# roym899/sdfest

Hardware: AMD Instinct MI355X
Metric: depth renders/sec fwd+bwd, 640×480 @ 64³ SDF; grad max-abs-err vs ref (higher is better)
Workload: dtype f32

## Files before the change

sdfest_amd/csrc/device.hpp:

```cpp
#pragma once

#include "common.hpp"

namespace sdfr {
namespace {

__device__ __forceinline__ V3 pixel_ray(int row, int col, float cx, float cy, float rfx, float rfy) {
  const float dx = ((float)col + 0.5f - cx) * rfx;
  const float dy = -((float)row + 0.5f - cy) * rfy;
  const float inv_len = __builtin_amdgcn_rsqf(fmaf(dx, dx, fmaf(dy, dy, 1.0f)));
  return mk(dx * inv_len, dy * inv_len, -inv_len);
}

__device__ __forceinline__ V3 rot_t(const ViewSetup& s, V3 v) {
  return mk(fmaf(s.rot[0], v.x, fmaf(s.rot[3], v.y, s.rot[6] * v.z)),
            fmaf(s.rot[1], v.x, fmaf(s.rot[4], v.y, s.rot[7] * v.z)),
            fmaf(s.rot[2], v.x, fmaf(s.rot[5], v.y, s.rot[8] * v.z)));
}
__device__ __forceinline__ V3 rot_f(const ViewSetup& s, V3 v) {
  return mk(fmaf(s.rot[0], v.x, fmaf(s.rot[1], v.y, s.rot[2] * v.z)),
            fmaf(s.rot[3], v.x, fmaf(s.rot[4], v.y, s.rot[5] * v.z)),
            fmaf(s.rot[6], v.x, fmaf(s.rot[7], v.y, s.rot[8] * v.z)));
}

__device__ __forceinline__ float vmin(float a, float b) {
  float r;
  asm("v_min_f32 %0, %1, %2" : "=v"(r) : "v"(a), "v"(b));
  return r;
}
__device__ __forceinline__ float vmax(float a, float b) {
  float r;
  asm("v_max_f32 %0, %1, %2" : "=v"(r) : "v"(a), "v"(b));
  return r;
}

struct __attribute__((packed, aligned(4))) ZPair {
  float lo, hi;
};

struct Cell {
  float v[8];
  float ox, oy, oz;
  float bx, by, bz;
  int lin;
};

template <int RT>
__device__ __forceinline__ void gather_cell(const float* __restrict__ src, int R, float gx, float gy,
                                            float gz, Cell& c) {
  const int Rr = RT > 0 ? RT : R;
  const float top = (float)(Rr - 2);
  const float bx = fminf(fmaxf(floorf(gx), 0.0f), top);
  const float by = fminf(fmaxf(floorf(gy), 0.0f), top);
  const float bz = fminf(fmaxf(floorf(gz), 0.0f), top);
  c.ox = gx - bx; c.oy = gy - by; c.oz = gz - bz;
  c.bx = bx; c.by = by; c.bz = bz;
  const int lin = (Rr <= 256) ? (int)fmaf(fmaf(bx, (float)Rr, by), (float)Rr, bz)
                              : ((int)bx * Rr + (int)by) * Rr + (int)bz;
  c.lin = lin;
  const float* base = src + lin;
  const ZPair p00 = *reinterpret_cast<const ZPair*>(base);
  const ZPair p01 = *reinterpret_cast<const ZPair*>(base + Rr);
  const ZPair p10 = *reinterpret_cast<const ZPair*>(base + Rr * Rr);
  const ZPair p11 = *reinterpret_cast<const ZPair*>(base + Rr * Rr + Rr);
  c.v[0] = p00.lo; c.v[1] = p00.hi; c.v[2] = p01.lo; c.v[3] = p01.hi;
  c.v[4] = p10.lo; c.v[5] = p10.hi; c.v[6] = p11.lo; c.v[7] = p11.hi;
}

constexpr bool kRecordsBlocked = true;
__host__ __device__ __forceinline__ int record_slab(int R) {
  return kRecordsBlocked ? 4 * ((R + 1) >> 1) * ((R + 1) >> 1) : R * R;
}
__device__ __forceinline__ int record_index(int x, int y, int z, int Hb) {
  if (!kRecordsBlocked) return (x * (2 * Hb) + y) * (2 * Hb) + z;
  return (((x * Hb + (y >> 1)) * Hb + (z >> 1)) << 2) | ((y & 1) << 1) | (z & 1);
}

typedef int i32x4 __attribute__((ext_vector_type(4)));

typedef float f32x2 __attribute__((ext_vector_type(2)));
typedef int i32x2 __attribute__((ext_vector_type(2)));
__host__ __device__ __forceinline__ constexpr bool is_pow2(int v) { return v > 0 && (v & (v - 1)) == 0; }

template <int RT, bool PACKED>
__device__ __forceinline__ float march_sample(__amdgpu_buffer_rsrc_t src, int R, f32x2 gxy, float gz) {
  const int Rr = RT > 0 ? RT : R;
  const float top = (float)(Rr - 2), fR = (float)Rr;
  const f32x2 bxy = {fminf(fmaxf(floorf(gxy.x), 0.0f), top), fminf(fmaxf(floorf(gxy.y), 0.0f), top)};
  const float bz = fminf(fmaxf(floorf(gz), 0.0f), top);
  const f32x2 oxy = gxy - bxy, axy = 1.0f - oxy;
  const float oz = gz - bz, az = 1.0f - oz;
  const int lin = (Rr <= 256) ? (int)fmaf(fmaf(bxy.x, fR, bxy.y), fR, bz)
                              : ((int)bxy.x * Rr + (int)bxy.y) * Rr + (int)bz;
  f32x2 a01, a23, b01, b23;
  if (PACKED) {
    int rix;
    if (!kRecordsBlocked) {
      rix = lin;
    } else if (RT > 0 && is_pow2(RT) && RT >= 4) {
      constexpr int L = __builtin_ctz(RT > 0 ? RT : 2);
      constexpr int zhi = ((1 << L) - 2) << 1;
      int t;
      asm("v_bfi_b32 %0, %1, %2, %3" : "=v"(t) : "s"(zhi), "v"(lin << 1), "v"(lin));
      asm("v_bfi_b32 %0, 2, %1, %2" : "=v"(rix) : "v"(lin >> (L - 1)), "v"(t));
    } else {
      rix = record_index((int)bxy.x, (int)bxy.y, (int)bz, (Rr + 1) >> 1);
    }
    const i32x4 a = __builtin_amdgcn_raw_buffer_load_b128(src, rix * 16, 0, 0);
    const i32x4 b = __builtin_amdgcn_raw_buffer_load_b128(src, rix * 16, record_slab(Rr) * 16, 0);
    a01 = f32x2{__int_as_float(a.x), __int_as_float(a.y)};
    a23 = f32x2{__int_as_float(a.z), __int_as_float(a.w)};
    b01 = f32x2{__int_as_float(b.x), __int_as_float(b.y)};
    b23 = f32x2{__int_as_float(b.z), __int_as_float(b.w)};
  } else {
    const int off = lin * 4;
    const i32x2 p00 = __builtin_amdgcn_raw_buffer_load_b64(src, off, 0, 0);
    const i32x2 p01 = __builtin_amdgcn_raw_buffer_load_b64(src, off, Rr * 4, 0);
    const i32x2 p10 = __builtin_amdgcn_raw_buffer_load_b64(src, off, Rr * Rr * 4, 0);
    const i32x2 p11 = __builtin_amdgcn_raw_buffer_load_b64(src, off, (Rr * Rr + Rr) * 4, 0);
    a01 = f32x2{__int_as_float(p00.x), __int_as_float(p00.y)};
    a23 = f32x2{__int_as_float(p01.x), __int_as_float(p01.y)};
    b01 = f32x2{__int_as_float(p10.x), __int_as_float(p10.y)};
    b23 = f32x2{__int_as_float(p11.x), __int_as_float(p11.y)};
  }
  const f32x2 ox2 = {oxy.x, oxy.x}, ax2 = {axy.x, axy.x}, oy2 = {oxy.y, oxy.y}, ay2 = {axy.y, axy.y};
  const f32x2 c0 = __builtin_elementwise_fma(b01, ox2, a01 * ax2);
  const f32x2 c1 = __builtin_elementwise_fma(b23, ox2, a23 * ax2);
  const f32x2 c = __builtin_elementwise_fma(c1, oy2, c0 * ay2);
  return fmaf(c.y, oz, c.x * az);
}

__device__ __forceinline__ float trilerp(const Cell& c) {
  const float ax = 1.0f - c.ox, ay = 1.0f - c.oy, az = 1.0f - c.oz;
  const float c00 = fmaf(c.v[4], c.ox, c.v[0] * ax);
  const float c01 = fmaf(c.v[5], c.ox, c.v[1] * ax);
  const float c10 = fmaf(c.v[6], c.ox, c.v[2] * ax);
  const float c11 = fmaf(c.v[7], c.ox, c.v[3] * ax);
  const float c0 = fmaf(c10, c.oy, c00 * ay);
  const float c1 = fmaf(c11, c.oy, c01 * ay);
  return fmaf(c1, c.oz, c0 * az);
}

constexpr int kPatchWFwd = 8, kPatchWBwd = 16;
template <int PW> struct Patch {
  static constexpr int W = PW, H = 64 / PW, waves_x = kSubW / PW;
  static __device__ __forceinline__ int ox(int wave) { return (wave % waves_x) * W; }
  static __device__ __forceinline__ int oy(int wave) { return (wave / waves_x) * H; }
  static __device__ __forceinline__ int x(int lane) { return lane % W; }
  static __device__ __forceinline__ int y(int lane) { return lane / W; }
};
__device__ __forceinline__ float wave_sum(float v) {
#pragma unroll
  for (int off = 32; off >= 1; off >>= 1) v += __shfl_xor(v, off, 64);
  return v;
}

__device__ __forceinline__ float wave_sum8(const float (&v)[8], int lane) {
  const bool b5 = lane & 32, b4 = lane & 16, b3 = lane & 8;
  float a[4], b[2], c;
#pragma unroll
  for (int j = 0; j < 4; ++j) {
    const float keep = b5 ? v[j + 4] : v[j], send = b5 ? v[j] : v[j + 4];
    a[j] = keep + __shfl_xor(send, 32, 64);
  }
#pragma unroll
  for (int j = 0; j < 2; ++j) {
    const float keep = b4 ? a[j + 2] : a[j], send = b4 ? a[j] : a[j + 2];
    b[j] = keep + __shfl_xor(send, 16, 64);
  }
  {
    const float keep = b3 ? b[1] : b[0], send = b3 ? b[0] : b[1];
    c = keep + __shfl_xor(send, 8, 64);
  }
  c += __shfl_xor(c, 4, 64);
  c += __shfl_xor(c, 2, 64);
  c += __shfl_xor(c, 1, 64);
  return c;
}

constexpr int kFixedBits = 44;

__device__ __forceinline__ long long fixed_from_float(float x) {
  const double d = (double)x + 6755399441055744.0;
  return __double_as_longlong(d) - 0x4338000000000000LL;
}

template <int SHIFT, int SLOTS>
struct RunHash {
  static constexpr int kShift = SHIFT, kSlots = SLOTS, kLen = 1 << SHIFT;
  static constexpr int kBits = kFixedBits;
  static constexpr float kWeightLimit = 3.5e13f;
  unsigned long long vals[SLOTS << SHIFT];
  int keys[SLOTS];

  __device__ __forceinline__ void clear(int tid, int nthreads) {
    for (int i = tid; i < SLOTS; i += nthreads) keys[i] = -1;
    for (int i = tid; i < (SLOTS << SHIFT); i += nthreads) vals[i] = 0ull;
  }

  __device__ __forceinline__ int slot_of(int key) {
    unsigned h = (((unsigned)key * 2654435761u) >> 16) & (SLOTS - 1);
#pragma unroll 1
    for (int probe = 0; probe < 32; ++probe) {
      int cur = __builtin_nontemporal_load(&keys[h]);
      if (cur == -1) cur = atomicCAS(&keys[h], -1, key);
      if (cur == -1 || cur == key) return (int)h;
      h = (h + 1) & (SLOTS - 1);
    }
    return -1;
  }

  template <bool DET = false>
  __device__ __forceinline__ void add_one(float* __restrict__ gvol, int slot, int lin, float w,
                                          float to_fixed) {
    if (slot >= 0)
      atomicAdd(&vals[(slot << SHIFT) + (lin & (kLen - 1))], (unsigned long long)fixed_from_float(w * to_fixed));
    else if (DET)
      atomicAdd(reinterpret_cast<unsigned long long*>(gvol) + lin, (unsigned long long)fixed_from_float(w * to_fixed));
    else
      atomicAdd(gvol + lin, w);
  }

  template <bool DET = false>
  __device__ __forceinline__ void add_cell(float* __restrict__ gvol, int lin, int Rr,
                                           const float (&w)[8], float to_fixed) {
    const int col[4] = {lin, lin + Rr, lin + Rr * Rr, lin + Rr * Rr + Rr};
    int key[4], cur[4];
    unsigned h[4];
#pragma unroll
    for (int j = 0; j < 4; ++j) {
      key[j] = col[j] >> SHIFT;
      h[j] = (((unsigned)key[j] * 2654435761u) >> 16) & (SLOTS - 1);
      cur[j] = __builtin_nontemporal_load(&keys[h[j]]);
    }
    int slot[4];
#pragma unroll
    for (int j = 0; j < 4; ++j) slot[j] = (cur[j] == key[j]) ? (int)h[j] : slot_of(key[j]);
#pragma unroll
    for (int j = 0; j < 4; ++j) {
      add_one<DET>(gvol, slot[j], col[j], w[2 * j], to_fixed);
      const bool split = (col[j] & (kLen - 1)) == kLen - 1;
      const int s_hi = split ? slot_of(key[j] + 1) : slot[j];
      add_one<DET>(gvol, s_hi, col[j] + 1, w[2 * j + 1], to_fixed);
    }
  }

  template <bool DET = false>
  __device__ __forceinline__ void flush(float* __restrict__ gvol, int nvox, float from_fixed, int tid,
                                        int nthreads) {
    for (int i = tid; i < (SLOTS << SHIFT); i += nthreads) {
      const int key = keys[i >> SHIFT];
      if (key < 0) continue;
      const long long q = (long long)vals[i];
      const int lin = (key << SHIFT) + (i & (kLen - 1));
      if (q != 0 && lin < nvox) {
        if (DET) atomicAdd(reinterpret_cast<unsigned long long*>(gvol) + lin, (unsigned long long)q);
        else atomicAdd(gvol + lin, (float)q * from_fixed);
      }
    }
  }
};
template <int SLOTS>
struct PairRunHash {
  static constexpr int kSlots = SLOTS, kLen = 4;
  static constexpr int kBits = 22;
  static constexpr float kWeightLimit = 4194304.0f;
  unsigned long long vals[SLOTS * 4];
  int keys[SLOTS];

  __device__ __forceinline__ void clear(int tid, int nthreads) {
    typedef int i32x4v __attribute__((ext_vector_type(4)));
    i32x4v* k4 = reinterpret_cast<i32x4v*>(keys);
    i32x4v* v4 = reinterpret_cast<i32x4v*>(vals);
    for (int i = tid; i < SLOTS / 4; i += nthreads) k4[i] = i32x4v{-1, -1, -1, -1};
    for (int i = tid; i < SLOTS * 2; i += nthreads) v4[i] = i32x4v{0, 0, 0, 0};
  }

  __device__ __forceinline__ int slot_after(int key, unsigned h, int cur) {
#pragma unroll 1
    for (int probe = 0; probe < 32; ++probe) {
      if (cur == -1) cur = atomicCAS(&keys[h], -1, key);
      if (cur == -1 || cur == key) return (int)h;
      h = (h + 1) & (SLOTS - 1);
      cur = __builtin_nontemporal_load(&keys[h]);
    }
    return -1;
  }

  template <bool DET = false>
  __device__ __forceinline__ void add_cell(float* __restrict__ gvol, int lin, int Rr, const float (&w)[8],
                                           float to_fixed) {
    static_assert(!DET, "32-bit pair sums cannot hold the deterministic mode's quantum: use RunHash");
    const int col[4] = {lin, lin + Rr, lin + Rr * Rr, lin + Rr * Rr + Rr};
    int key[4], cur[4];
    unsigned h[4];
#pragma unroll
    for (int j = 0; j < 4; ++j) {
      key[j] = col[j] >> 2;
      h[j] = (((unsigned)key[j] * 2654435761u) >> 16) & (SLOTS - 1);
      cur[j] = __builtin_nontemporal_load(&keys[h[j]]);
    }
    int slot[4];
#pragma unroll
    for (int j = 0; j < 4; ++j) slot[j] = (cur[j] == key[j]) ? (int)h[j] : slot_after(key[j], h[j], cur[j]);
#pragma unroll
    for (int j = 0; j < 4; ++j) {
      if (slot[j] >= 0) {
        const long long lo = fixed_from_float(w[2 * j] * to_fixed), hi = fixed_from_float(w[2 * j + 1] * to_fixed);
        atomicAdd(&vals[slot[j] * 4 + (col[j] & 3)], (unsigned long long)(lo + (hi << 32)));
      } else {
        atomicAdd(gvol + col[j], w[2 * j]);
        atomicAdd(gvol + col[j] + 1, w[2 * j + 1]);
      }
    }
  }

  template <bool DET = false>
  __device__ __forceinline__ void flush(float* __restrict__ gvol, int nvox, float from_fixed, int tid, int nthreads) {
    static_assert(!DET, "use RunHash");
    for (int i = tid; i < SLOTS * 5; i += nthreads) {
      const int slot = i / 5, k = i - slot * 5;
      const int key = keys[slot];
      if (key < 0) continue;
      long long sum = 0;
      if (k < 4) sum += (long long)(int)(unsigned)(vals[slot * 4 + k] & 0xffffffffull);
      if (k > 0) {
        const long long q = (long long)vals[slot * 4 + k - 1];
        sum += (q - (long long)(int)(unsigned)((unsigned long long)q & 0xffffffffull)) >> 32;
      }
      const int lin = key * 4 + k;
      if (sum != 0 && lin < nvox) atomicAdd(gvol + lin, (float)sum * from_fixed);
    }
  }
};
using BatchHash = RunHash<2, 512>;
using SmallHash = RunHash<1, 1024>;

template <int CTRL> __device__ __forceinline__ int dpp_self(int v) {
  return __builtin_amdgcn_update_dpp(v, v, CTRL, 0xf, 0xf, false);
}
__device__ __forceinline__ int wave_min_to63(int v) {
  v = min(v, dpp_self<0x111>(v));
  v = min(v, dpp_self<0x112>(v));
  v = min(v, dpp_self<0x114>(v));
  v = min(v, dpp_self<0x118>(v));
  v = min(v, dpp_self<0x142>(v));
  v = min(v, dpp_self<0x143>(v));
  return v;
}
__device__ __forceinline__ int wave_max_to63(int v) {
  v = max(v, dpp_self<0x111>(v));
  v = max(v, dpp_self<0x112>(v));
  v = max(v, dpp_self<0x114>(v));
  v = max(v, dpp_self<0x118>(v));
  v = max(v, dpp_self<0x142>(v));
  v = max(v, dpp_self<0x143>(v));
  return v;
}

__device__ __forceinline__ float wave_max(float v) {
#pragma unroll
  for (int off = 32; off >= 1; off >>= 1) v = fmaxf(v, __shfl_xor(v, off, 64));
  return v;
}


}
}
```

sdfest_amd/csrc/render.hip:

```cpp
#include <algorithm>
#include <atomic>
#include <type_traits>

#include "common.hpp"
#include "device.hpp"
#include "sampler_device.hpp"


namespace sdfr {
namespace {

constexpr int kBlock = 256;
constexpr int kFwdWaves = SDFR_FWD_WAVES;
constexpr int kInlineSetupMaxViews = SDFR_INLINE_MAX_VIEWS;


__device__ __forceinline__ void setup_pose(int b, const float* __restrict__ pos, const float* __restrict__ quat,
                                           const float* __restrict__ inv_scale, int R, float fx, float fy,
                                           ViewSetup& s) {
  const float x = quat[4 * b], y = quat[4 * b + 1], z = quat[4 * b + 2], w = quat[4 * b + 3];
  const V3 p = mk(pos[3 * b], pos[3 * b + 1], pos[3 * b + 2]);
  const float isc = inv_scale[b];
  const float scale = 1.0f / isc;
  s.rot[0] = 1 - 2 * (y * y + z * z); s.rot[1] = 2 * (x * y - w * z);     s.rot[2] = 2 * (x * z + w * y);
// ... 50 lines not shown
            const unsigned long long m = __ballot(f);
            if (m) {
              if (first == R) first = i0 + __builtin_ctzll(m);
              last = i0 + 63 - __builtin_clzll(m);
            }
          }
        } else {
          for (int i = 0; i + 1 < R; ++i) {
            if (fminf(pm[i], pm[i + 1]) < vhit) {
              if (first == R) first = i;
              last = i;
            }
          }
        }
        if (last < 0) { empty = true; break; }
        lo[a] = fmaxf(-scale, ((float)first - 0.0625f) * cell - scale);
        hi[a] = fminf(scale, ((float)(last + 1) + 0.0625f) * cell - scale);
      }
    }
  }
  float umin = 3.0e38f, umax = -3.0e38f, vmin = 3.0e38f, vmax = -3.0e38f;
  bool in_front = true;
  auto corner = [&](int c) {
    const float sx = (c & 1) ? hi[0] : lo[0], sy = (c & 2) ? hi[1] : lo[1],
                sz = (c & 4) ? hi[2] : lo[2];
    const float X = p.x + s.rot[0] * sx + s.rot[1] * sy + s.rot[2] * sz;
    const float Y = p.y + s.rot[3] * sx + s.rot[4] * sy + s.rot[5] * sz;
    const float Z = p.z + s.rot[6] * sx + s.rot[7] * sy + s.rot[8] * sz;
    if (!(Z < -1e-6f)) in_front = false;
    const float iz = 1.0f / fmaxf(-Z, 1e-30f);
    const float u = cx + fx * X * iz;
    const float v = cy - fy * Y * iz;
    umin = fminf(umin, u); umax = fmaxf(umax, u);
    vmin = fminf(vmin, v); vmax = fmaxf(vmax, v);
  };
  if (WAVE) {
    corner(lane & 7);
#pragma unroll
    for (int off = 1; off <= 4; off <<= 1) {
      umin = fminf(umin, __shfl_xor(umin, off, 64)); umax = fmaxf(umax, __shfl_xor(umax, off, 64));
      vmin = fminf(vmin, __shfl_xor(vmin, off, 64)); vmax = fmaxf(vmax, __shfl_xor(vmax, off, 64));
    }
    in_front = __ballot(!in_front) == 0ull;
  } else {
    for (int c = 0; c < 8; ++c) corner(c);
  }
  int x0 = 0, y0 = 0, x1 = W, y1 = H;
  if (in_front) {
    const float mx = 2.0f + 1e-5f * fabsf(fx), my = 2.0f + 1e-5f * fabsf(fy);
    const float fx0 = fminf(fmaxf(floorf(umin - 0.5f - mx), 0.0f), (float)W);
    const float fx1 = fminf(fmaxf(ceilf(umax - 0.5f + mx) + 1.0f, 0.0f), (float)W);
    const float fy0 = fminf(fmaxf(floorf(vmin - 0.5f - my), 0.0f), (float)H);
    const float fy1 = fminf(fmaxf(ceilf(vmax - 0.5f + my) + 1.0f, 0.0f), (float)H);
    x0 = (int)fx0; x1 = (int)fx1; y0 = (int)fy0; y1 = (int)fy1;
  }
  if (empty) { x0 = y0 = x1 = y1 = 0; }
  s.rect[0] = x0; s.rect[1] = y0; s.rect[2] = x1; s.rect[3] = y1;
  if (WAVE && spans) {
    float cu[8], cv[8];
    float big = 0.0f;
#pragma unroll
    for (int c = 0; c < 8; ++c) {
      const float sx = (c & 1) ? hi[0] : lo[0], sy = (c & 2) ? hi[1] : lo[1], sz = (c & 4) ? hi[2] : lo[2];
      const float X = p.x + s.rot[0] * sx + s.rot[1] * sy + s.rot[2] * sz;
      const float Y = p.y + s.rot[3] * sx + s.rot[4] * sy + s.rot[5] * sz;
      const float Z = p.z + s.rot[6] * sx + s.rot[7] * sy + s.rot[8] * sz;
      const float iz = 1.0f / fmaxf(-Z, 1e-30f);
      cu[c] = cx + fx * X * iz;
      cv[c] = cy - fy * Y * iz;
      big = fmaxf(big, fmaxf(fabsf(cu[c]), fabsf(cv[c])));
    }
    bool sane = in_front && !empty && big < 4.0e4f && W <= 65535;
#pragma unroll
    for (int c = 0; c < 8; ++c) sane = sane && (cu[c] == cu[c]) && (cv[c] == cv[c]);
    s.spans = sane ? 1 : 0;
    const int rstride = resident_stride_words(H);
    if (sane || rr.row) {
      const float mx = 2.0f + 1e-5f * fabsf(fx), my = 2.0f + 1e-5f * fabsf(fy);
      const int nb = span_bands(H);
      float slope[12];
#pragma unroll
      for (int a = 0, e = 0; a < 8; ++a)
#pragma unroll
        for (int ax = 0; ax < 3; ++ax)
          if (!(a & (1 << ax))) {
            const int c2 = a | (1 << ax);
            slope[e++] = (cu[c2] - cu[a]) * __builtin_amdgcn_rcpf(cv[c2] - cv[a]);
          }
      for (int k0 = 0; k0 < nb; k0 += 64) {
        const int k = k0 + lane;
        const float ya = (float)(8 * k) + 0.5f - my, yb = (float)(8 * k) + 7.5f + my;
        float xmin = 3.0e38f, xmax = -3.0e38f;
        float da[8], db[8];
#pragma unroll
        for (int a = 0; a < 8; ++a) {
          da[a] = ya - cv[a];
          db[a] = yb - cv[a];
          const float u = (da[a] <= 0.0f && db[a] >= 0.0f) ? cu[a] : __int_as_float(0x7fc00000);
          xmin = fminf(xmin, u); xmax = fmaxf(xmax, u);
        }
#pragma unroll
        for (int a = 0, e = 0; a < 8; ++a)
#pragma unroll
          for (int ax = 0; ax < 3; ++ax)
            if (!(a & (1 << ax))) {
              const int c2 = a | (1 << ax);
              const float xa = (da[a] * da[c2] <= 0.0f) ? fmaf(da[a], slope[e], cu[a]) : __int_as_float(0x7fc00000);
              const float xb = (db[a] * db[c2] <= 0.0f) ? fmaf(db[a], slope[e], cu[a]) : __int_as_float(0x7fc00000);
              xmin = fminf(xmin, fminf(xa, xb)); xmax = fmaxf(xmax, fmaxf(xa, xb));
              ++e;
            }
        int sx0 = 0, sx1 = 0;
        if (!sane) {
          if (x1 > x0 && 8 * k < y1 && 8 * k + 8 > y0) { sx0 = x0; sx1 = x1; }
        } else if (xmin <= xmax && 8 * k < y1 && 8 * k + 8 > y0) {
          sx0 = max(x0, (int)fminf(fmaxf(floorf(xmin - 0.5f - mx), 0.0f), (float)W));
          sx1 = min(x1, (int)fminf(fmaxf(ceilf(xmax - 0.5f + mx) + 1.0f, 0.0f), (float)W));
          if (sx1 <= sx0) sx0 = sx1 = 0;
        }
        const unsigned word = (unsigned)sx0 | ((unsigned)sx1 << 16);
        if (k < nb) {
          if (sane) spans[k] = word;
          if (rr.row) {
            const unsigned prev = !rr.prev_ok ? kResidentClearAll : (k0 == 0 ? rr.prev0 : rr.row[2 * k]);
            rr.row[2 * k] = word;
            rr.row[2 * k + 1] = prev;
          }
        }
      }
      if (rr.row && lane == 0) {
        rr.row[rstride - 2] = rr.seq + 1u;
        rr.row[rstride - 1] = ~((rr.seq + 1u) ^ rr.key);
      }
    }
  }
  for (int k = 0; k < 3; ++k) {
    s.ep[k] = s.e[k] + scale;
    s.em[k] = s.e[k] - scale;
    s.tp[k] = s.e[k] + hi[k];
    s.tm[k] = s.e[k] + lo[k];
  }
}

template <bool WAVE = false>
__device__ __forceinline__ void compute_view_setup(int b, const float* __restrict__ pos,
                                                   const float* __restrict__ quat,
                                                   const float* __restrict__ inv_scale, int R, int W, int H,
                                                   float cx, float cy, float fx, float fy,
                                                   ViewSetup* __restrict__ out,
                                                   const float* __restrict__ plane_min = nullptr,
                                                   float threshold = 0.0f, unsigned* __restrict__ spans = nullptr,
                                                   ResidentRow rr = ResidentRow{}) {
  ViewSetup s;
  setup_pose(b, pos, quat, inv_scale, R, fx, fy, s);
  setup_box<WAVE>(s, R, W, H, cx, cy, fx, fy, plane_min, threshold,
                  spans ? spans + (size_t)b * span_stride_words(H) : nullptr, rr);
  if (!WAVE || (threadIdx.x & 63) == 0) out[b] = s;
}

__device__ __forceinline__ void count_close_view(unsigned* __restrict__ sync, int B, bool close,
                                                 unsigned long long* __restrict__ word) {
  const unsigned old = atomicAdd(&sync[2], 0x10000u | (close ? 1u : 0u));
  if ((old >> 16) + 1u != (unsigned)B) return;
  const unsigned c = (old & 0xffffu) + (close ? 1u : 0u);
  atomicExch(&sync[2], 0u);
  const unsigned seq = sync[4] + 1u;
  sync[4] = seq;
  sync[5] = c;
  if (word) __hip_atomic_store(word, ((unsigned long long)seq << 32) | c, __ATOMIC_RELAXED, __HIP_MEMORY_SCOPE_SYSTEM);
}

__device__ __forceinline__ ResidentRow resident_row(unsigned* __restrict__ rstate, int vouched, int b, int B, int W,
                                                    int H) {
  ResidentRow rr;
  if (rstate) {
    const int stride = resident_stride_words(H), lane = threadIdx.x & 63;
    rr.row = rstate + kResidentHeaderWords + (size_t)b * stride;
    rr.seq = rstate[0];
    rr.key = resident_key(B, W, H);
    const unsigned tag = rr.row[stride - 2], check = rr.row[stride - 1];
    rr.prev0 = lane < span_bands(H) ? rr.row[2 * lane] : 0u;
    rr.prev_ok = vouched != 0 && tag == rr.seq && check == ~(rr.seq ^ rr.key);
  }
  return rr;
}

__global__ void view_setup_kernel(const float* __restrict__ pos, const float* __restrict__ quat,
                                  const float* __restrict__ inv_scale, int B, int R, int W, int H,
                                  float cx, float cy, float fx, float fy,
                                  ViewSetup* __restrict__ out, const float* __restrict__ plane_min,
                                  float threshold, unsigned* __restrict__ spans, unsigned* __restrict__ rstate,
                                  int depth_resident) {
  const int b = blockIdx.x;
  if (b < B)
    compute_view_setup<true>(b, pos, quat, inv_scale, R, W, H, cx, cy, fx, fy, out, plane_min, threshold, spans,
                             resident_row(rstate, depth_resident, b, B, W, H));
}

struct PlaneEntry {
  unsigned long long a, b;
};
__device__ __forceinline__ void publish_plane_min(float* __restrict__ plane_min, PlaneEntry* __restrict__ ent,
                                                  unsigned tag, int j, float m) {
  if (ent) {
    const unsigned bits = __float_as_uint(m);
    __hip_atomic_store(&ent[j].a, ((unsigned long long)tag << 32) | bits, __ATOMIC_RELAXED, __HIP_MEMORY_SCOPE_AGENT);
    __hip_atomic_store(&ent[j].b, ((unsigned long long)tag << 32) | (unsigned)~bits, __ATOMIC_RELAXED,
                       __HIP_MEMORY_SCOPE_AGENT);
  } else {
    plane_min[j] = m;
  }
}

__device__ __forceinline__ void plane_min_block(const float* __restrict__ sdf, int R, int j,
                                                float* __restrict__ plane_min, PlaneEntry* __restrict__ ent = nullptr,
                                                unsigned tag = 0u) {
  __shared__ float red[4][4];
  const int axis = j / R, i = j % R, RR = R * R;
  const int tid = threadIdx.x;
  if (axis == 2 && (R & 3) == 0 && ((uintptr_t)sdf & 15) == 0) {
    if (i & 3) return;
    float m0 = 3.0e38f, m1 = 3.0e38f, m2 = 3.0e38f, m3 = 3.0e38f;
    for (int k = tid; k < RR; k += 256) {
      const float4 v = *reinterpret_cast<const float4*>(sdf + (size_t)k * R + i);
      m0 = fminf(m0, v.x); m1 = fminf(m1, v.y); m2 = fminf(m2, v.z); m3 = fminf(m3, v.w);
    }
#pragma unroll
    for (int off = 32; off >= 1; off >>= 1) {
      m0 = fminf(m0, __shfl_xor(m0, off, 64)); m1 = fminf(m1, __shfl_xor(m1, off, 64));
      m2 = fminf(m2, __shfl_xor(m2, off, 64)); m3 = fminf(m3, __shfl_xor(m3, off, 64));
    }
    if ((tid & 63) == 0) { red[tid >> 6][0] = m0; red[tid >> 6][1] = m1; red[tid >> 6][2] = m2; red[tid >> 6][3] = m3; }
    __syncthreads();
    if (tid < 4)
      publish_plane_min(plane_min, ent, tag, j + tid,
                        fminf(fminf(red[0][tid], red[1][tid]), fminf(red[2][tid], red[3][tid])));
    return;
  }
  float m = 3.0e38f;
  for (int k = tid; k < RR; k += 256) {
    const int u = k / R, v = k % R;
    const int idx = axis == 0 ? i * RR + k : (axis == 1 ? u * RR + i * R + v : k * R + i);
    m = fminf(m, sdf[idx]);
  }
#pragma unroll
  for (int off = 32; off >= 1; off >>= 1) m = fminf(m, __shfl_xor(m, off, 64));
  if ((tid & 63) == 0) red[tid >> 6][0] = m;
  __syncthreads();
  if (tid == 0) publish_plane_min(plane_min, ent, tag, j, fminf(fminf(red[0][0], red[1][0]), fminf(red[2][0], red[3][0])));
}

__global__ __launch_bounds__(256) void backward_prologue_kernel(
    float* __restrict__ g_sdf, size_t n_words, const float* __restrict__ pos,
    const float* __restrict__ quat, const float* __restrict__ inv_scale, int B, int R, int W, int H,
    float cx, float cy, float fx, float fy, ViewSetup* __restrict__ out) {
  const size_t i = (size_t)blockIdx.x * 256 + threadIdx.x;
  if (i < n_words) g_sdf[i] = 0.0f;
  if (i < (size_t)B) compute_view_setup((int)i, pos, quat, inv_scale, R, W, H, cx, cy, fx, fy, out);
}

__device__ __forceinline__ float4 min4(float4 a, float4 b) {
  return make_float4(fminf(a.x, b.x), fminf(a.y, b.y), fminf(a.z, b.z), fminf(a.w, b.w));
}
__device__ __forceinline__ void plane_min_fast_block(const float* __restrict__ sdf, int R, int blk,
                                                     PlaneEntry* __restrict__ ent, unsigned tag) {
  __shared__ float4 red4[4];
  const int tid = threadIdx.x, RR = R * R, Rq = R >> 2;
  const float4* v = reinterpret_cast<const float4*>(sdf);
  float4 m = make_float4(3.0e38f, 3.0e38f, 3.0e38f, 3.0e38f);
  const int axis = blk / R, i = blk - axis * R;
  if (axis == 0) {
    const float4* base = v + (size_t)i * (RR >> 2);
#pragma unroll 4
    for (int q = tid; q < (RR >> 2); q += 256) m = min4(m, base[q]);
  } else if (axis == 1) {
    const float4* base = v + (size_t)i * Rq;
#pragma unroll 4
    for (int q = tid; q < R * Rq; q += 256) m = min4(m, base[(size_t)(q / Rq) * (RR >> 2) + (q % Rq)]);
  } else {
    const int zq = i % Rq, part = i / Rq, rows = RR >> 2;
    const float4* base = v + (size_t)part * rows * Rq + zq;
#pragma unroll 4
    for (int r = tid; r < rows; r += 256) m = min4(m, base[(size_t)r * Rq]);
  }
#pragma unroll
  for (int off = 32; off >= 1; off >>= 1) {
    m.x = fminf(m.x, __shfl_xor(m.x, off, 64)); m.y = fminf(m.y, __shfl_xor(m.y, off, 64));
    m.z = fminf(m.z, __shfl_xor(m.z, off, 64)); m.w = fminf(m.w, __shfl_xor(m.w, off, 64));
  }
  if ((tid & 63) == 0) red4[tid >> 6] = m;
  __syncthreads();
  if (tid < 4) {
    const float4 a = min4(min4(red4[0], red4[1]), min4(red4[2], red4[3]));
    if (axis < 2) {
      if (tid == 0) publish_plane_min(nullptr, ent, tag, blk, fminf(fminf(a.x, a.y), fminf(a.z, a.w)));
    } else {
      const int zq = i % Rq, part = i / Rq;
      const float val = tid == 0 ? a.x : (tid == 1 ? a.y : (tid == 2 ? a.z : a.w));
      publish_plane_min(nullptr, ent, tag, 2 * R + part * R + 4 * zq + tid, val);
    }
  }
}

__device__ __forceinline__ void pack_cell(const float* __restrict__ sdf, int R, float4* __restrict__ cells, int lin) {
  const int RR = R * R;
  if (lin >= RR * R) return;
  const int z = lin % R, y = (lin / R) % R;
  if (y >= R - 1 || z >= R - 1) return;
  const float* p = sdf + lin;
  cells[record_index(lin / RR, y, z, (R + 1) >> 1)] = make_float4(p[0], p[1], p[R], p[R + 1]);
}

__global__ __launch_bounds__(256) void pack_cells_kernel(const float* __restrict__ sdf, int R,
                                                         float4* __restrict__ cells, int n_pack_blocks,
                                                         float* __restrict__ plane_min) {
  const int n_plane = (int)gridDim.x - n_pack_blocks;
  if ((int)blockIdx.x < n_plane) {
    plane_min_block(sdf, R, (int)blockIdx.x, plane_min);
    return;
  }
  pack_cell(sdf, R, cells, ((int)blockIdx.x - n_plane) * (int)blockDim.x + (int)threadIdx.x);
}

constexpr int kPrologueMaxPolls = 1 << 16;
__global__ __launch_bounds__(256) void forward_prologue_kernel(
    const float* __restrict__ sdf, int R, float4* __restrict__ cells, int n_plane, int n_setup,
    unsigned* __restrict__ sync, const float* __restrict__ pos, const float* __restrict__ quat,
    const float* __restrict__ inv_scale, int B, int W, int H, float cx, float cy, float fx, float fy,
    ViewSetup* __restrict__ out, float threshold, float* __restrict__ g_zero, size_t n_zero, int default_polls,
    unsigned* __restrict__ spans, unsigned* __restrict__ rstate, int depth_resident) {
  const unsigned tag = sync[0] + 1u;
  PlaneEntry* ent = reinterpret_cast<PlaneEntry*>(sync + kSyncHeaderWords);
  int blk = (int)blockIdx.x;
  if (blk < n_plane) {
    plane_min_fast_block(sdf, R, blk, ent, tag);
    return;
  }
  blk -= n_plane;
  if (blk < n_setup) {
    __shared__ float pm_s[6 * kPackedMaxR];
    const int tid = (int)threadIdx.x, n_ent = 6 * R;
    const int b = blk * 4 + (tid >> 6);
    ViewSetup s;
    ResidentRow rr;
    if (b < B) {
      setup_pose(b, pos, quat, inv_scale, R, fx, fy, s);
      rr = resident_row(rstate, depth_resident, b, B, W, H);
    }
    bool ready = false;
    const int max_polls = sync[6] == SDFR_SYNC_POLLS_MAGIC ? (int)sync[7] : default_polls;
    for (int poll = 0; poll < max_polls; ++poll) {
      bool ok = true;
      for (int j = tid; j < n_ent; j += 256) {
        const unsigned long long a = __hip_atomic_load(&ent[j].a, __ATOMIC_RELAXED, __HIP_MEMORY_SCOPE_AGENT);
        const unsigned long long c = __hip_atomic_load(&ent[j].b, __ATOMIC_RELAXED, __HIP_MEMORY_SCOPE_AGENT);
        const bool good = (unsigned)(a >> 32) == tag && (unsigned)(c >> 32) == tag && (unsigned)a == ~(unsigned)c;
        if (good) pm_s[j] = __uint_as_float((unsigned)a);
        ok = ok && good;
      }
      if (__syncthreads_and(ok)) { ready = true; break; }
      __builtin_amdgcn_s_sleep(1);
    }
    if (ready) {
      for (int z = tid; z < R; z += 256)
        pm_s[2 * R + z] = fminf(fminf(pm_s[2 * R + z], pm_s[3 * R + z]), fminf(pm_s[4 * R + z], pm_s[5 * R + z]));
      __syncthreads();
    }
    if (b < B) {
      setup_box<true>(s, R, W, H, cx, cy, fx, fy, ready ? pm_s : nullptr, threshold,
                      spans + (size_t)b * span_stride_words(H), rr);
      if ((tid & 63) == 0) {
        out[b] = s;
        if (!ready) atomicAdd(&sync[1], 1u);
      }
    }
    return;
  }
  blk -= n_setup;
  const int lin = blk * 256 + (int)threadIdx.x;
  const size_t vox = (size_t)R * R * R;
  for (size_t i = (size_t)lin; i < n_zero; i += vox) g_zero[i] = 0.0f;
  pack_cell(sdf, R, cells, lin);
}

struct Rect {
  int x0, y0, x1, y1;
};
__device__ __forceinline__ bool overlaps(const Rect& r, int px, int py, int w, int h) {
  return (px < r.x1) && (px + w > r.x0) && (py < r.y1) && (py + h > r.y0);
}

struct Ray {
  float dg[3];
  float t, tf;
  float inv_len;
  bool go;
};
template <bool TIGHT>
__device__ __forceinline__ Ray ray_setup(const ViewSetup& s, int row, int col, bool inside, float cx, float cy,
                                         float rfx, float rfy) {
  Ray r;
  const float dx = ((float)col + 0.5f - cx) * rfx;
  const float dy = -((float)row + 0.5f - cy) * rfy;
  const float inv_len = __builtin_amdgcn_rsqf(fmaf(dx, dx, fmaf(dy, dy, 1.0f)));
  const float ux = fmaf(s.rot[0], dx, fmaf(s.rot[3], dy, -s.rot[6]));
  const float uy = fmaf(s.rot[1], dx, fmaf(s.rot[4], dy, -s.rot[7]));
  const float uz = fmaf(s.rot[2], dx, fmaf(s.rot[5], dy, -s.rot[8]));
  const float dv[3] = {ux * inv_len, uy * inv_len, uz * inv_len};
  float t_near = -1e-10f, tf = 1e10f, t_near2 = -1e-10f, tf2 = 1e10f;
#pragma unroll
  for (int a = 0; a < 3; ++a) {
    const float inv = __builtin_amdgcn_rcpf(dv[a]);
    const float ta = s.ep[a] * inv, tb = s.em[a] * inv;
    t_near = vmax(t_near, vmin(ta, tb));
    if (TIGHT) {
      const float tc = s.tp[a] * inv, td = s.tm[a] * inv;
      t_near2 = vmax(t_near2, vmin(tc, td));
      tf2 = vmin(tf2, vmax(tc, td));
    } else {
      tf = vmin(tf, vmax(ta, tb));
    }
  }
  if (TIGHT) tf = tf2;
  const bool miss = !inside || (TIGHT ? ((t_near2 > tf2) || (tf2 < 0.0f)) : ((t_near > tf) || (tf < 0.0f)));
  r.t = vmax(t_near, 0.0f);
  r.tf = tf;
  r.inv_len = inv_len;
  r.go = !miss && (r.t < tf);
  const float kgrid = s.dgk;
  r.dg[0] = dv[0] * kgrid; r.dg[1] = dv[1] * kgrid; r.dg[2] = dv[2] * kgrid;
  return r;
}

template <int RT, bool PACKED, int SX, int SY, bool LOSS, bool TIGHT, int NW, bool RES = false>
__device__ __forceinline__ void forward_tile(
    int tile_x, int tile_y, int ntx, int nty, int b, const float* __restrict__ src, int R,
    long long src_view_stride, const ViewSetup& s, int W, int H, float cx, float cy,
    float rfx, float rfy, float threshold, int vec_ok, float* __restrict__ depth,
    const float* __restrict__ target, float* __restrict__ loss_part, const unsigned* __restrict__ spans,
    const unsigned* __restrict__ rrows = nullptr) {
  constexpr int kSubs = SX * SY, kTileW = SX * kSubW, kTileH = SY * kSubH;
  static_assert(kTileH == 8, "a forward tile is one band of the span array");
  constexpr int kThreads = NW * 64;
  using PF = Patch<kPatchWFwd>;
  const int px0 = tile_x * kTileW, py0 = tile_y * kTileH;
  float* img = depth + (size_t)b * H * W;
  const int tid = threadIdx.x;
  auto zero_fill = [&]() {
    typedef float f32x4 __attribute__((ext_vector_type(4)));
    const f32x4 zero4 = {0.0f, 0.0f, 0.0f, 0.0f};
    if (vec_ok) {
#pragma unroll
      for (int i = tid; i < kTileW * kTileH / 4; i += kThreads) {
        const int row = py0 + i / (kTileW / 4), col = px0 + (i % (kTileW / 4)) * 4;
        if (row < H && col < W) __builtin_nontemporal_store(zero4, reinterpret_cast<f32x4*>(img + (size_t)row * W + col));
      }
    } else {
      for (int i = tid; i < kTileW * kTileH; i += kThreads) {
        const int row = py0 + i / kTileW, col = px0 + i % kTileW;
        if (row < H && col < W) img[(size_t)row * W + col] = 0.0f;
      }
    }
  };
  uint2 band = make_uint2(0u, kResidentClearAll);
  if (RES && rrows) {
    band = *reinterpret_cast<const uint2*>(rrows + (size_t)b * resident_stride_words(H) + 2 * tile_y);
    if (!LOSS && !(px0 < (int)(band.x >> 16) && px0 + kTileW > (int)(band.x & 0xffffu))) {
      if (px0 < (int)(band.y >> 16) && px0 + kTileW > (int)(band.y & 0xffffu)) zero_fill();
      return;
    }
  }
  Rect rc{s.rect[0], s.rect[1], s.rect[2], s.rect[3]};
  const bool in_rect = overlaps(rc, px0, py0, kTileW, kTileH);
  if (RES && rrows) {
    rc.x0 = (int)(band.x & 0xffffu);
    rc.x1 = (int)(band.x >> 16);
  } else if (s.spans) {
    const unsigned sp = spans[(size_t)b * span_stride_words(H) + tile_y];
    rc.x0 = (int)(sp & 0xffffu);
    rc.x1 = (int)(sp >> 16);
  }

  if (!overlaps(rc, px0, py0, kTileW, kTileH)) {
    if (LOSS && in_rect && tid < kLossRec) loss_part[(((size_t)b * nty + tile_y) * ntx + tile_x) * kLossRec + tid] = 0.0f;
    if (px0 < (int)(band.y >> 16) && px0 + kTileW > (int)(band.y & 0xffffu)) zero_fill();
    return;
  }

  const int wave = tid >> 6, lane = tid & 63;
  const float scale = s.scale;
  const float* vol = src + (size_t)b * src_view_stride;
  const int Rr = RT > 0 ? RT : R;
  const unsigned src_bytes = PACKED ? (unsigned)Rr * record_slab(Rr) * 16u : (unsigned)Rr * Rr * Rr * 4u;
  const __amdgpu_buffer_rsrc_t vsrc =
      __builtin_amdgcn_make_buffer_rsrc(const_cast<float*>(vol), 0, (int)src_bytes, 0x00020000);

  float l_sum = 0.0f, l_cnt = 0.0f;
  const float* obs = LOSS ? target + (size_t)b * H * W : nullptr;
  const float og[3] = {s.og[0], s.og[1], s.og[2]};
  for (int it = wave; it < 4 * kSubs; it += NW) {
    const int sub = it >> 2, pw = it & 3;
    const int sx = px0 + (sub % SX) * kSubW, sy = py0 + (sub / SX) * kSubH;
    const int col = sx + PF::ox(pw) + PF::x(lane), row = sy + PF::oy(pw) + PF::y(lane);
    const bool inside = (col < W) && (row < H);
    float result = 0.0f;
    if (overlaps(rc, sx + PF::ox(pw), sy + PF::oy(pw), PF::W, PF::H)) {
      const Ray r = ray_setup<TIGHT>(s, row, col, inside, cx, cy, rfx, rfy);
      if (r.go) {
        const f32x2 dgxy = {r.dg[0], r.dg[1]}, ogxy = {og[0], og[1]};
        float t = r.t;
        bool hit;
        int n = 0;
        for (;;) {
          ++n;
          const f32x2 t2 = {t, t};
          const float value = march_sample<RT, PACKED>(vsrc, R, __builtin_elementwise_fma(t2, dgxy, ogxy),
                                                       fmaf(t, r.dg[2], og[2]));
          const float dist = value * scale;
          hit = dist < threshold * t;
          if (hit) break;
          const float tn = t + dist;
          if (!(tn < r.tf) || n >= SDFR_MAX_MARCH_STEPS) break;
          t = tn;
        }
        result = hit ? t * r.inv_len : 0.0f;
        if (LOSS && result > 0.0f) {
          const float o = obs[row * W + col];
          if (o > 0.0f) {
            l_sum += fabsf(result - o);
            l_cnt += 1.0f;
          }
        }
      }
    }
    if (inside) img[row * W + col] = result;
  }
  if (LOSS) {
    l_sum = wave_sum(l_sum);
    l_cnt = wave_sum(l_cnt);
    float* rec = loss_part + (((size_t)b * nty + tile_y) * ntx + tile_x) * kLossRec;
    if (lane == 0) *reinterpret_cast<float2*>(rec + 2 * wave) = make_float2(l_sum, l_cnt);
    if (NW < 4 && wave == 0 && lane >= 2 * NW && lane < kLossRec) rec[lane] = 0.0f;
  }
}

struct InlineSetup {
  const float* pos;
  const float* quat;
  const float* inv_scale;
  float fx, fy;
  ViewSetup* out;
  float* g_zero;
  size_t n_zero;
};
template <int RT, bool PACKED, int SX, int SY, bool LOSS, int NW, bool INLINE = false, bool RES = false>
__global__ __launch_bounds__(NW * 64) void render_forward_kernel(
    const float* __restrict__ src, int R, long long src_view_stride,
    const ViewSetup* __restrict__ setup, int W, int H, int ntx, int nty, float cx, float cy,
    float rfx, float rfy, float threshold, int vec_ok, float* __restrict__ depth,
    const float* __restrict__ target, float* __restrict__ loss_part, unsigned* __restrict__ epoch,
    const unsigned* __restrict__ spans, InlineSetup in, unsigned* __restrict__ count_sync,
    unsigned long long* __restrict__ close_word, const unsigned* __restrict__ rrows, unsigned* __restrict__ rseq) {
  if (INLINE) {
    const int b = blockIdx.z;
    ViewSetup s;
    setup_pose(b, in.pos, in.quat, in.inv_scale, R, in.fx, in.fy, s);
    setup_box<false>(s, R, W, H, cx, cy, in.fx, in.fy, nullptr, threshold);
    if ((blockIdx.x | blockIdx.y) == 0 && threadIdx.x == 0) in.out[b] = s;
    const size_t nthreads = (size_t)gridDim.x * gridDim.y * gridDim.z * (NW * 64);
    const size_t me = (((size_t)b * gridDim.y + blockIdx.y) * gridDim.x + blockIdx.x) * (NW * 64) + threadIdx.x;
    for (size_t i = me; i < in.n_zero; i += nthreads) in.g_zero[i] = 0.0f;
    forward_tile<RT, PACKED, SX, SY, LOSS, PACKED, NW>(blockIdx.x, blockIdx.y, ntx, nty, b, src, R, src_view_stride,
                                                       s, W, H, cx, cy, rfx, rfy, threshold, vec_ok, depth, target,
                                                       loss_part, spans);
    if (rseq && (blockIdx.x | blockIdx.y | blockIdx.z) == 0 && threadIdx.x == 0) rseq[0] += 1u;
    return;
  }
  forward_tile<RT, PACKED, SX, SY, LOSS, PACKED, NW, RES>(blockIdx.x, blockIdx.y, ntx, nty, blockIdx.z, src, R,
                                         src_view_stride, setup[blockIdx.z], W, H, cx, cy, rfx, rfy, threshold,
                                         vec_ok, depth, target, loss_part, spans, rrows);
  if (rseq && (blockIdx.x | blockIdx.y | blockIdx.z) == 0 && threadIdx.x == 0) rseq[0] += 1u;
  if (count_sync && (blockIdx.x | blockIdx.y) == 0 && threadIdx.x == 0)
    count_close_view(count_sync, (int)gridDim.z, setup[blockIdx.z].bwd_big != 0, close_word);
  if (epoch && (blockIdx.x | blockIdx.y | blockIdx.z) == 0) {
    if (threadIdx.x == 0) epoch[0] += 1u;
    unsigned long long* ent = reinterpret_cast<unsigned long long*>(epoch + kSyncHeaderWords);
    for (int j = threadIdx.x; j < 2 * 6 * kPackedMaxR; j += NW * 64) ent[j] = 0ull;
  }
}

constexpr int kDenseCap = SDFR_DENSE_CAP;

template <typename Hash>
struct BackwardLds {
  union {
    Hash hash;
    int dense[kDenseCap > 0 ? kDenseCap : 4];
  };
  float wave_part[4][8];
  int tile_max_bits;
  int box[6];
  float loss_pair[4][2];
};

__host__ __device__ constexpr int tile_fixed_bits(int pixels, int table_bits) {
  int b = 31;
  for (int p = 1; p < pixels; p <<= 1) --b;
  return b < table_bits ? b : table_bits;
}
template <typename Hash> struct HashIs32 { static constexpr bool value = false; };
template <int SLOTS> struct HashIs32<PairRunHash<SLOTS>> { static constexpr bool value = true; };

struct HitPoint {
// ... 1287 lines not shown
```

Baseline: 1.030 million.

## Reorder packed cell records so x-neighbor record sits adjacent

Changes the blocked record layout so the x index varies fastest within each 2x2 (y,z) block, placing the x+1 neighbour record a fixed 4 records (64 bytes) away instead of a full slab away. The two 128-bit loads per trilinear sample then hit nearby memory, which should improve cache-line locality. The pow2 fast path computes the new index with a float FMA plus bitfield ops, and the packing kernel now iterates over record indices instead of voxel indices. The fast path is limited to R<=64, and the packing now reads the source SDF with a different access pattern.

```diff
diff --git a/sdfest_amd/csrc/device.hpp b/sdfest_amd/csrc/device.hpp
--- a/sdfest_amd/csrc/device.hpp
+++ b/sdfest_amd/csrc/device.hpp
@@ -67,14 +67,12 @@
   c.v[4] = p10.lo; c.v[5] = p10.hi; c.v[6] = p11.lo; c.v[7] = p11.hi;
 }
 
-constexpr bool kRecordsBlocked = true;
-__host__ __device__ __forceinline__ int record_slab(int R) {
-  return kRecordsBlocked ? 4 * ((R + 1) >> 1) * ((R + 1) >> 1) : R * R;
-}
-__device__ __forceinline__ int record_index(int x, int y, int z, int Hb) {
-  if (!kRecordsBlocked) return (x * (2 * Hb) + y) * (2 * Hb) + z;
-  return (((x * Hb + (y >> 1)) * Hb + (z >> 1)) << 2) | ((y & 1) << 1) | (z & 1);
-}
+__host__ __device__ __forceinline__ int record_slab(int R) { return 4 * ((R + 1) >> 1) * ((R + 1) >> 1); }
+__host__ __device__ __forceinline__ int record_index(int x, int y, int z, int R) {
+  const int Hyz = R >> 1, X2 = ((R + 1) >> 1) * 2;
+  return (((((y >> 1) * Hyz + (z >> 1)) * X2 + x) << 2) | ((y & 1) << 1)) | (z & 1);
+}
+constexpr int kRecordNextX = 4;
 
 typedef int i32x4 __attribute__((ext_vector_type(4)));
 
@@ -95,19 +93,18 @@
   f32x2 a01, a23, b01, b23;
   if (PACKED) {
     int rix;
-    if (!kRecordsBlocked) {
-      rix = lin;
-    } else if (RT > 0 && is_pow2(RT) && RT >= 4) {
+    if (RT > 0 && is_pow2(RT) && RT >= 4 && RT <= 64) {
       constexpr int L = __builtin_ctz(RT > 0 ? RT : 2);
-      constexpr int zhi = ((1 << L) - 2) << 1;
+      constexpr int from_w = (((1 << L) - 1) << 2) | (((1 << (L - 1)) - 1) << (2 * L + 1));
+      const int w = (int)fmaf(bz, (float)(1 << (3 * L)), fmaf(bxy.y, (float)(1 << (2 * L)), bxy.x * 4.0f));
       int t;
-      asm("v_bfi_b32 %0, %1, %2, %3" : "=v"(t) : "s"(zhi), "v"(lin << 1), "v"(lin));
-      asm("v_bfi_b32 %0, 2, %1, %2" : "=v"(rix) : "v"(lin >> (L - 1)), "v"(t));
+      asm("v_bfi_b32 %0, %1, %2, %3" : "=v"(t) : "s"(from_w), "v"(w), "v"(w >> (2 * L - 1)));
+      rix = t + (int)__builtin_amdgcn_ubfe(w, 3 * L, 1);
     } else {
-      rix = record_index((int)bxy.x, (int)bxy.y, (int)bz, (Rr + 1) >> 1);
+      rix = record_index((int)bxy.x, (int)bxy.y, (int)bz, Rr);
     }
     const i32x4 a = __builtin_amdgcn_raw_buffer_load_b128(src, rix * 16, 0, 0);
-    const i32x4 b = __builtin_amdgcn_raw_buffer_load_b128(src, rix * 16, record_slab(Rr) * 16, 0);
+    const i32x4 b = __builtin_amdgcn_raw_buffer_load_b128(src, rix * 16 + kRecordNextX * 16, 0, 0);
     a01 = f32x2{__int_as_float(a.x), __int_as_float(a.y)};
     a23 = f32x2{__int_as_float(a.z), __int_as_float(a.w)};
     b01 = f32x2{__int_as_float(b.x), __int_as_float(b.y)};
diff --git a/sdfest_amd/csrc/render.hip b/sdfest_amd/csrc/render.hip
--- a/sdfest_amd/csrc/render.hip
+++ b/sdfest_amd/csrc/render.hip
@@ -376,13 +376,13 @@
   }
 }
 
-__device__ __forceinline__ void pack_cell(const float* __restrict__ sdf, int R, float4* __restrict__ cells, int lin) {
-  const int RR = R * R;
-  if (lin >= RR * R) return;
-  const int z = lin % R, y = (lin / R) % R;
-  if (y >= R - 1 || z >= R - 1) return;
-  const float* p = sdf + lin;
-  cells[record_index(lin / RR, y, z, (R + 1) >> 1)] = make_float4(p[0], p[1], p[R], p[R + 1]);
+__device__ __forceinline__ void pack_cell(const float* __restrict__ sdf, int R, float4* __restrict__ cells, int rix) {
+  const int Hyz = R >> 1, X2 = ((R + 1) >> 1) * 2;
+  const int q = rix >> 2, x = q % X2, b = q / X2;
+  const int y = (b / Hyz) * 2 + ((rix >> 1) & 1), z = (b % Hyz) * 2 + (rix & 1);
+  if (x >= R || y >= R - 1 || z >= R - 1) return;
+  const float* p = sdf + ((size_t)x * R + y) * R + z;
+  cells[rix] = make_float4(p[0], p[1], p[R], p[R + 1]);
 }
 
 __global__ __launch_bounds__(256) void pack_cells_kernel(const float* __restrict__ sdf, int R,
```

Measured after the change: 1.056 million, median of 6. 1.02x the previous value.
